# jerryli27/TwinGAN

Hardware: AMD Instinct MI355X
Metric: training images/sec (G+D step) at 256×256 final stage, 1/2/4/8 MI355X (higher is better)
Workload: dtype bf16; 1 GPU; TwinGAN 256x256 stage, batch 16 per GPU (configs[3]): E/G/2xD max_ch 256, UNet + per-domain instance norm + pixel norm, WGAN-GP, Adam; 1 step = G apply + D apply; global_batch=16, batch_per_gpu=16, parallelism=dp1, launch=hipGraph replay

## Files before the change

twingan_amd/csrc/norm.hip:

```cpp
#include "tg_common.h"
#include <stdlib.h>
#include <type_traits>

namespace {

#ifndef TG_NORM_BWD_U
#define TG_NORM_BWD_U 2
#endif
#define NF_LRELU 1
#define NF_PIXNORM 2
#define NF_ZEROSHIFT 8
#define NF_NOSTATS 4

template <typename T, int V>
struct VecIO {
  __device__ static __forceinline__ void load(const T* p, float* o) {
    if constexpr (V == 1) {
      o[0] = ld(p);
    } else {
      Vec16<T> v = ldv(p);
#pragma unroll
      for (int j = 0; j < V; ++j) o[j] = v.get(j);
    }
  }
// ... 447 lines not shown
        for (int q = 0; q < U; ++q) {
          const bool live = !TAIL || pb + q * lanes < p1;
          float yh[V];
          norm_act_gu<V>(gq[q], xq[q], sq[q], mu, rs, ga, be, flags, alpha, cv, inv_c, yh);
#pragma unroll
          for (int j = 0; j < V; ++j) {
            const float gr = live ? gq[q][j] : 0.f;
            a1[j] += gr;
            a2[j] = fmaf(gr, yh[j], a2[j]);
          }
        }
      }
    };
    if ((p1 - p0) % (lanes * U) == 0) sweep(std::false_type());
    else sweep(std::true_type());
  }
  wave_channel_accumulate<V>(a1, sh, 0, cv, v, pl < lanes);
  wave_channel_accumulate<V>(a2, sh, c, cv, v, pl < lanes);
  __syncthreads();
  float* out = sums + ((int64_t)n * gridDim.x + blockIdx.x) * 2 * c;
  for (int i = threadIdx.x; i < 2 * c; i += blockDim.x) out[i] = sh[i];
}

template <typename T, int V, int FL = -1>
__global__ void norm_act_bwd2_part_kernel(const T* __restrict__ gz, const T* __restrict__ gzp, int wdim,
                                          const T* __restrict__ y, const float* __restrict__ pn_scale,
                                          const float* __restrict__ mean, const float* __restrict__ rstd,
                                          const float* __restrict__ gamma, const float* __restrict__ beta,
                                          const float* __restrict__ gamma2, const float* __restrict__ beta2, int split,
                                          int pstride, T* __restrict__ gy, const float* __restrict__ part, int chunks,
                                          float* __restrict__ ggamma, float* __restrict__ gbeta,
                                          float* __restrict__ ggamma2, float* __restrict__ gbeta2, int sink, int hw, int c,
                                          int flags_rt, float alpha, int px_per_block) {
  extern __shared__ float sh[];
  const int flags = FL < 0 ? flags_rt : ((flags_rt & ~3) | FL);
  const int cv = c / V;
  const int lanes = blockDim.x / cv;
  const int v = threadIdx.x % cv, pl = threadIdx.x / cv;
  const int n = blockIdx.y;
  float mu[V], rs[V], ga[V], be[V];
#pragma unroll
  for (int j = 0; j < V; ++j) {
    const int ch = v * V + j;
    mu[j] = mean[n * c + ch];
    rs[j] = rstd[n * c + ch];
    ga[j] = pstride ? gamma[(int64_t)n * pstride + ch] : (n < split ? gamma : gamma2)[ch];
    be[j] = pstride ? beta[(int64_t)n * pstride + ch] : (n < split ? beta : beta2)[ch];
  }
  reduce_partials<exact_path<T>()>(part, n, chunks, c, sh);
  if (pstride && blockIdx.x == 0) {
    for (int i = threadIdx.x; i < c; i += blockDim.x) {
      if (gbeta) gbeta[(int64_t)n * pstride + i] = sh[i];
      if (ggamma) ggamma[(int64_t)n * pstride + i] = sh[c + i];
    }
  } else if (sink && blockIdx.x == 0) {
    float* gg = n < split ? ggamma : ggamma2;
    float* gb = n < split ? gbeta : gbeta2;
    if (sink == 2) {
      const int i0 = n < split ? 0 : split, i1 = n < split ? split : (int)gridDim.y;
      if (n == i0) {
        for (int i = threadIdx.x; i < 2 * c; i += blockDim.x) {
          float t = 0.f;
          const int64_t k1 = (int64_t)i1 * chunks;
          int64_t k = (int64_t)i0 * chunks;
          for (; k + 8 <= k1; k += 8) {
            float v[8];
#pragma unroll
            for (int u = 0; u < 8; ++u) v[u] = part[(k + u) * 2 * c + i];
#pragma unroll
            for (int u = 0; u < 8; ++u) t += v[u];
          }
          for (; k < k1; ++k) t += part[k * 2 * c + i];
          float* dst = i < c ? gb : gg;
          if (dst) atomicAdd(dst + (i < c ? i : i - c), t);
        }
      }
    } else {
      for (int i = threadIdx.x; i < c; i += blockDim.x) {
        if (gb) atomicAdd(gb + i, sh[i]);
        if (gg) atomicAdd(gg + i, sh[c + i]);
      }
    }
  }
  const float inv = 1.f / (float)hw;
  float s1[V], s2[V];
#pragma unroll
  for (int j = 0; j < V; ++j) {
    const int ch = v * V + j;
    s1[j] = (flags & NF_NOSTATS) ? 0.f : sh[ch] * inv;
    s2[j] = (flags & NF_NOSTATS) ? 0.f : sh[c + ch] * inv;
  }
  const int p0 = blockIdx.x * px_per_block;
  const int p1 = min(p0 + px_per_block, hw);
  if (pl >= lanes) return;
  const T* gz_n = gz ? gz + (int64_t)n * hw * c : nullptr;
  const T* gzp_n = gzp ? gzp + (int64_t)n * (hw >> 2) * c : nullptr;
  const T* y_n = y + (int64_t)n * hw * c;
  T* gy_n = gy + (int64_t)n * hw * c;
  const float* pn_n = pn_scale ? pn_scale + (int64_t)n * hw : nullptr;
  const int wshift = (wdim & (wdim - 1)) == 0 ? 31 - __builtin_clz(wdim) : -1;
  float gr[V];
#pragma unroll
  for (int j = 0; j < V; ++j) gr[j] = ga[j] * rs[j];
  const float inv_c = 1.f / (float)c;
  constexpr int U = TG_NORM_BWD_U;
  auto sweep = [&](auto tail) __attribute__((always_inline)) {
    constexpr bool TAIL = decltype(tail)::value;
    for (int pb = p0 + pl; pb < p1; pb += lanes * U) {
      float gq[U][V], xq[U][V], sq[U];
#pragma unroll
      for (int q = 0; q < U; ++q) {
        const unsigned p = TAIL ? min(pb + q * lanes, p1 - 1) : pb + q * lanes;
        load_grad_img<T, V>(gz_n, gzp_n, p, wshift, wdim, c, v, 0.25f, gq[q]);
        VecIO<T, V>::load(y_n + (p * c + v * V), xq[q]);
        sq[q] = (flags & NF_PIXNORM) ? pn_n[p] : 1.f;
      }
#pragma unroll
      for (int q = 0; q < U; ++q) {
        const unsigned p = pb + q * lanes;
        float yh[V];
        norm_act_gu<V>(gq[q], xq[q], sq[q], mu, rs, ga, be, flags, alpha, cv, inv_c, yh);
#pragma unroll
        for (int j = 0; j < V; ++j) gq[q][j] = gr[j] * (gq[q][j] - s1[j] - yh[j] * s2[j]);
        if (!TAIL || p < (unsigned)p1) VecIO<T, V>::store_stream(gy_n, p * c + v * V, gq[q]);
      }
    }
  };
  if ((p1 - p0) % (lanes * U) == 0) sweep(std::false_type());
  else sweep(std::true_type());
}

__global__ void norm_param_grads(const float* __restrict__ part, int chunks, float* __restrict__ ggamma,
                                 float* __restrict__ gbeta, float* __restrict__ ggamma2, float* __restrict__ gbeta2,
                                 int split, int n, int c, int accumulate) {
  const int ch = blockIdx.x * blockDim.x + threadIdx.x;
  if (ch >= c) return;
  const int i0 = blockIdx.y ? split : 0, i1 = blockIdx.y ? n : split;
  float* gg = blockIdx.y ? ggamma2 : ggamma;
  float* gb = blockIdx.y ? gbeta2 : gbeta;
  float sb = 0.f, sg = 0.f;
  for (int64_t k = (int64_t)i0 * chunks; k < (int64_t)i1 * chunks; ++k) {
    sb += part[k * 2 * c + ch];
    sg += part[k * 2 * c + c + ch];
  }
  if (gg) {
    if (accumulate) atomicAdd(gg + ch, sg);
    else gg[ch] = sg;
  }
  if (gb) {
    if (accumulate) atomicAdd(gb + ch, sb);
    else gb[ch] = sb;
  }
// ... 326 lines not shown
  norm_chunks(n, hw, &chunks, &ppb);
  int chunks2 = (2048 + n - 1) / n;
  int ppb2 = (hw + chunks2 - 1) / chunks2;
  if (ppb2 < min_ppb(hw)) ppb2 = min_ppb(hw);
  chunks2 = (hw + ppb2 - 1) / ppb2;
  const bool want_params = ggamma || gbeta || ggamma2 || gbeta2;
  TG_CHECK(!pstride || !accumulate, TG_EINVAL, "tg_norm_act_bwd: per-image parameter gradients are written, not added");
  int sink = (want_params && accumulate) ? 1 : 0;
  const size_t lds = 2 * (size_t)c * sizeof(float);
  TG_DISPATCH_DTYPE(dtype, "tg_norm_act_bwd", {
    if (sink && exact_grid<T>()) sink = 2;
    constexpr int VN = Vec16<T>::N;
    const bool vec = (c % VN == 0) && pow2(c / VN) && c / VN <= 64;
    if (flags & NF_PIXNORM) {
      TG_CHECK(vec && pn_scale, TG_ENOSUP, "tg_norm_act_bwd: pixel norm needs c (%d) = %d * 2^k and pn_scale", c, VN);
    }
    if (vec) {
      switch (flags & 3) {
        case 0: TG_NB_LAUNCH(0); break;
        case 1: TG_NB_LAUNCH(1); break;
        case 2: TG_NB_LAUNCH(2); break;
        default: TG_NB_LAUNCH(3); break;
      }
    } else {
      TG_CHECK(c <= 256, TG_ENOSUP, "tg_norm_act_bwd: scalar path needs c <= 256 (got %d)", c);
      hipLaunchKernelGGL((norm_act_bwd1_kernel<T, 1>), dim3(chunks, n), dim3(256), lds, s, (const T*)gz,
                         (const T*)gz_pooled, w, (const T*)y, pn_scale, mean, rstd, gamma, beta, gamma2, beta2, split, pstride, sums, hw, c, flags, alpha, ppb);
      hipLaunchKernelGGL((norm_act_bwd2_part_kernel<T, 1>), dim3(chunks2, n), dim3(256), lds, s, (const T*)gz,
                         (const T*)gz_pooled, w, (const T*)y, pn_scale, mean, rstd, gamma, beta, gamma2, beta2, split,
                         pstride, (T*)gy, sums, chunks, ggamma, gbeta, ggamma2, gbeta2, sink, hw, c, flags, alpha, ppb2);
    }
  });
  if (want_params && !sink && !pstride)
    hipLaunchKernelGGL(norm_param_grads, dim3((c + 255) / 256, split < n ? 2 : 1), dim3(256), 0, s, sums, chunks, ggamma,
                       gbeta, ggamma2, gbeta2, split, n, c, 0);
  TG_LAUNCH_CHECK("tg_norm_act_bwd");
  return TG_OK;
}

static int lrelu_bwd_launch(const char* who, const void* gz, const void* gzp, int hw, int wdim, const void* z, void* gy,
                            float* gbias, int64_t npix, int c, float alpha, int accumulate, int dtype, hipStream_t s,
                            bool z_is_sign_bits = false) {
  if (gbias && !accumulate) {
    int rc = tg_zero_async(gbias, (size_t)c * sizeof(float), nullptr, 0, s);
    if (rc) return rc;
  }
// ... 110 lines not shown
```

twingan_amd/csrc/pointwise.hip:

```cpp
#include "tg_common.h"

namespace {

template <typename T>
__global__ void axpby_kernel(const T* __restrict__ x, const T* __restrict__ y, T* __restrict__ out, int64_t numel, float a,
                             float b) {
  constexpr int V = Vec16<T>::N;
  const int64_t nvec = numel / V;
  const int64_t stride = (int64_t)gridDim.x * blockDim.x;
  for (int64_t i = (int64_t)blockIdx.x * blockDim.x + threadIdx.x; i < nvec; i += stride) {
    Vec16<T> vx = ldv(x + i * V), vo;
    if (y) {
      Vec16<T> vy = ldv(y + i * V);
#pragma unroll
      for (int j = 0; j < V; ++j) vo.set(j, a * vx.get(j) + b * vy.get(j));
    } else {
#pragma unroll
      for (int j = 0; j < V; ++j) vo.set(j, a * vx.get(j));
    }
    stv(out + i * V, vo);
  }
  for (int64_t i = nvec * V + (int64_t)blockIdx.x * blockDim.x + threadIdx.x; i < numel; i += stride)
    st(out + i, a * ld(x + i) + (y ? b * ld(y + i) : 0.f));
}
// ... 135 lines not shown
template <typename TS, typename TD>
__global__ void cast_kernel(const TS* __restrict__ s, TD* __restrict__ d, int64_t numel) {
  const int64_t stride = (int64_t)gridDim.x * blockDim.x;
  for (int64_t i = (int64_t)blockIdx.x * blockDim.x + threadIdx.x; i < numel; i += stride) st(d + i, ld(s + i));
}

template <typename T>
__global__ void sample_lerp_kernel(const T* __restrict__ x, const T* __restrict__ y, const float* __restrict__ alpha,
                                   T* __restrict__ out, int64_t per, int64_t numel) {
  const int64_t stride = (int64_t)gridDim.x * blockDim.x;
  for (int64_t i = (int64_t)blockIdx.x * blockDim.x + threadIdx.x; i < numel; i += stride) {
    const float a = alpha[i / per], vx = ld(x + i);
    st(out + i, vx + a * (ld(y + i) - vx));
  }
}

template <typename T>
__global__ void sample_scale_kernel(const T* __restrict__ x, const float* __restrict__ coef,
                                    const float* __restrict__ scalar, T* __restrict__ out, int64_t per, int64_t numel) {
  const int64_t stride = (int64_t)gridDim.x * blockDim.x;
  const float sc = scalar ? scalar[0] : 1.f;
  for (int64_t i = (int64_t)blockIdx.x * blockDim.x + threadIdx.x; i < numel; i += stride)
    st(out + i, ld(x + i) * coef[i / per] * sc);
}

template <typename T>
__global__ void gdrop_kernel(const T* __restrict__ x, const float* __restrict__ noise, const float* __restrict__ strength_dev,
                             float strength, float sqrt_c, T* __restrict__ out, int64_t per_image, int c, int64_t numel) {
  const int64_t stride = (int64_t)gridDim.x * blockDim.x;
  const float coef = (strength_dev ? strength_dev[0] : strength) * sqrt_c;
  for (int64_t i = (int64_t)blockIdx.x * blockDim.x + threadIdx.x; i < numel; i += stride) {
    const int64_t img = i / per_image;
    const int ch = (int)(i % c);
    st(out + i, ld(x + i) * fmaf(noise[img * c + ch], coef, 1.f));
  }
}

template <typename T, int V>
__global__ void upsample_concat_fwd_kernel(const T* __restrict__ x0, const T* __restrict__ x1, T* __restrict__ out, int n,
                                           int h, int w, int c0, int c1, int gsz, unsigned perm) {
  const int c = c0 + c1, cv = c / V, c0v = c0 / V;
  const int64_t total = (int64_t)n * (2 * h) * (2 * w) * cv;
  for (int64_t i = (int64_t)blockIdx.x * blockDim.x + threadIdx.x; i < total; i += (int64_t)gridDim.x * blockDim.x) {
    const int v = (int)(i % cv);
    int64_t p = i / cv;
    const int ox = (int)(p % (2 * w));
// ... 682 lines not shown
  else {
    tg_set_error("tg_cast: unsupported dtypes %d -> %d", sd, dd);
    return TG_EINVAL;
  }
  TG_LAUNCH_CHECK("tg_cast");
  return TG_OK;
}

int tg_sample_lerp(const void* x, const void* y, const float* alpha, void* out, int batch, int64_t per, int dtype,
                   void* stream) {
  TG_CHECK(x && y && alpha && out && batch > 0 && per > 0, TG_EINVAL, "tg_sample_lerp: bad arguments");
  TG_DISPATCH_DTYPE(dtype, "tg_sample_lerp", {
    hipLaunchKernelGGL(sample_lerp_kernel<T>, dim3(tg_grid_for(batch * per, 256)), dim3(256), 0, (hipStream_t)stream,
                       (const T*)x, (const T*)y, alpha, (T*)out, per, batch * per);
  });
  TG_LAUNCH_CHECK("tg_sample_lerp");
  return TG_OK;
}

int tg_sample_scale(const void* x, const float* coef, const float* scalar, void* out, int batch, int64_t per, int dtype,
                    void* stream) {
  TG_CHECK(x && coef && out && batch > 0 && per > 0, TG_EINVAL, "tg_sample_scale: bad arguments");
  TG_DISPATCH_DTYPE(dtype, "tg_sample_scale", {
    hipLaunchKernelGGL(sample_scale_kernel<T>, dim3(tg_grid_for(batch * per, 256)), dim3(256), 0, (hipStream_t)stream,
                       (const T*)x, coef, scalar, (T*)out, per, batch * per);
  });
  TG_LAUNCH_CHECK("tg_sample_scale");
  return TG_OK;
}

int tg_gdrop(const void* x, const float* noise, const float* strength_dev, float strength, int c_logical, void* out, int n,
             int64_t hw, int c, int dtype, void* stream) {
  TG_CHECK(x && noise && out && n > 0 && hw > 0 && c > 0 && c_logical > 0 && c_logical <= c, TG_EINVAL, "tg_gdrop: bad arguments");
  const int64_t per = hw * c;
  TG_DISPATCH_DTYPE(dtype, "tg_gdrop", {
    hipLaunchKernelGGL(gdrop_kernel<T>, dim3(tg_grid_for(n * per, 256)), dim3(256), 0, (hipStream_t)stream, (const T*)x, noise,
                       strength_dev, strength, sqrtf((float)c_logical), (T*)out, per, c, n * per);
  });
  TG_LAUNCH_CHECK("tg_gdrop");
  return TG_OK;
}

#define TG_SPATIAL_LAUNCH(KERNEL, VECOK, TOTAL_VEC, TOTAL_SCALAR, ...)                                                 \
  TG_DISPATCH_DTYPE(dtype, #KERNEL, {                                                                                  \
    constexpr int V = Vec16<T>::N;                                                                                     \
    if (VECOK(V))                                                                                                      \
      hipLaunchKernelGGL((KERNEL<T, V>), dim3(tg_grid_for(TOTAL_VEC(V), 256)), dim3(256), 0, (hipStream_t)stream,      \
                         __VA_ARGS__);                                                                                 \
// ... 149 lines not shown
```

twingan_amd/csrc/reduce.hip:

```cpp
#include "tg_common.h"

namespace {

constexpr int MB_NMAX = 16;
template <typename T, int V>
struct alignas(sizeof(T) * V) MbVec {
  T e[V];
  __device__ __forceinline__ float get(int i) const { return (float)e[i]; }
  __device__ __forceinline__ void set(int i, float x) { e[i] = (T)x; }
};
template <typename T> constexpr int mb_v() { return 8 / (int)sizeof(T); }
template <typename T, int V> __device__ __forceinline__ MbVec<T, V> mb_ld(const T* p) {
  return *reinterpret_cast<const MbVec<T, V>*>(p);
}
template <typename T, int V> __device__ __forceinline__ void mb_st(T* p, const MbVec<T, V>& v) {
  *reinterpret_cast<MbVec<T, V>*>(p) = v;
}
template <typename T, int V>
__device__ __forceinline__ void mb_load_samples(const T* __restrict__ x, int n, int P, int p, MbVec<T, V> (&xv)[MB_NMAX]) {
#pragma unroll
  for (int i = 0; i < MB_NMAX; ++i) xv[i] = mb_ld<T, V>(x + (int64_t)(i < n ? i : n - 1) * P + p);
}


// ... 348 lines not shown
      mb_copy_with_stat<T, 9>(v, ggout, total / V16, c, cpad, Tt);
    } else {
      for (int64_t i = threadIdx.x; i < total; i += blockDim.x) {
        const int ch = (int)(i % cpad);
        const int64_t px = i / cpad;
        float o = 0.f;
        if (ch < c)
          o = ld(v + px * c + ch);
        else if (ch == c)
          o = Tt;
        st(ggout + i, o);
      }
    }
  }
}

template <typename T, int MODE, bool PART = false>
__global__ void sum_kernel(const T* __restrict__ x, const T* __restrict__ y, float* __restrict__ out, int64_t numel,
                           float scale, int direct = 0, int vec = 1) {
  __shared__ float red[8];
  constexpr int V = Vec16<T>::N;
  const int64_t nvec = vec ? numel / V : 0, stride = (int64_t)gridDim.x * blockDim.x;
  float acc = 0.f;
  for (int64_t i = (int64_t)blockIdx.x * blockDim.x + threadIdx.x; i < nvec; i += stride) {
    Vec16<T> a = ldv(x + i * V);
    if (MODE == 0) {
#pragma unroll
      for (int j = 0; j < V; ++j) acc += a.get(j);
    } else {
      Vec16<T> b = ldv(y + i * V);
#pragma unroll
      for (int j = 0; j < V; ++j) acc += fabsf(a.get(j) - b.get(j));
    }
  }
  for (int64_t i = nvec * V + (int64_t)blockIdx.x * blockDim.x + threadIdx.x; i < numel; i += stride)
    acc += MODE == 0 ? ld(x + i) : fabsf(ld(x + i) - ld(y + i));
  const float tot = block_sum(acc, red);
  if (threadIdx.x == 0) {
    if constexpr (PART) out[blockIdx.x] = tot;
    else if (direct) out[0] = tot * scale;
    else atomicAdd(out, tot * scale);
  }
}

__global__ void ordered_scalar_sum_kernel(const float* __restrict__ part, int n, float* __restrict__ out, float scale,
                                          int accumulate) {
  if (blockIdx.x || threadIdx.x) return;
  float t = 0.f;
  for (int i = 0; i < n; ++i) t += part[i];
  out[0] = accumulate ? out[0] + t * scale : t * scale;
}

template <typename T>
__global__ void abs_diff_bwd_kernel(const T* __restrict__ a, const T* __restrict__ b, const float* __restrict__ gscale,
                                    T* __restrict__ ga, T* __restrict__ gb, int64_t numel, float scale) {
  const float g = (gscale ? gscale[0] : 1.f) * scale;
  for (int64_t i = (int64_t)blockIdx.x * blockDim.x + threadIdx.x; i < numel; i += (int64_t)gridDim.x * blockDim.x) {
    const float d = ld(a + i) - ld(b + i);
    const float s = d > 0.f ? g : (d < 0.f ? -g : 0.f);
    if (ga) st(ga + i, s);
    if (gb) st(gb + i, -s);
  }
}

template <typename T>
__global__ void sample_sumsq_kernel(const T* __restrict__ x, float* __restrict__ out, int64_t per, int vec) {
  __shared__ float red[8];
  constexpr int V = Vec16<T>::N;
  const T* base = x + (int64_t)blockIdx.y * per;
  const int64_t nvec = vec ? per / V : 0, stride = (int64_t)gridDim.x * blockDim.x;
  float acc = 0.f;
  for (int64_t i = (int64_t)blockIdx.x * blockDim.x + threadIdx.x; i < nvec; i += stride) {
    Vec16<T> a = ldv(base + i * V);
#pragma unroll
    for (int j = 0; j < V; ++j) acc = fmaf(a.get(j), a.get(j), acc);
  }
  for (int64_t i = nvec * V + (int64_t)blockIdx.x * blockDim.x + threadIdx.x; i < per; i += stride) {
    const float a = ld(base + i);
    acc = fmaf(a, a, acc);
  }
  const float tot = block_sum(acc, red);
  if (threadIdx.x == 0) atomicAdd(out + blockIdx.y, tot);
}

__global__ void gp_penalty_kernel(const float* __restrict__ ss, float* __restrict__ loss, float* __restrict__ coef,
                                  int batch, float lambda) {
  __shared__ float red[8];
  float acc = 0.f;
  for (int b = threadIdx.x; b < batch; b += blockDim.x) {
    const float slope = sqrtf(ss[b]);
    const float d = slope - 1.f;
    acc += d * d;
    if (coef) coef[b] = slope > 0.f ? lambda * 2.f * d / (slope * (float)batch) : 0.f;
  }
  const float tot = block_sum(acc, red);
  if (threadIdx.x == 0 && loss) loss[0] = lambda * tot / (float)batch;
}

// ... 147 lines not shown
template <typename T>
__global__ void fc_bwd_kernel(const T* __restrict__ x, const float* __restrict__ w, const float* __restrict__ g,
                              T* __restrict__ gx, float* __restrict__ gw, float* __restrict__ gb, int m, int n, int k,
                              int acc_w, int acc_b) {
  const int kk = blockIdx.x * blockDim.x + threadIdx.x;
  if (kk < k) {
    for (int row = 0; gx && row < m; ++row) {
      float a = 0.f;
      for (int col = 0; col < n; ++col) a = fmaf(g[(int64_t)row * n + col], w[(int64_t)kk * n + col], a);
      st(gx + (int64_t)row * k + kk, a);
    }
    for (int col = 0; gw && col < n; ++col) {
      float a = 0.f;
      for (int row = 0; row < m; ++row) a = fmaf(ld(x + (int64_t)row * k + kk), g[(int64_t)row * n + col], a);
      gw[(int64_t)kk * n + col] = (acc_w ? gw[(int64_t)kk * n + col] : 0.f) + a;
    }
  }
  if (gb && kk < n) {
    float a = 0.f;
    for (int row = 0; row < m; ++row) a += g[(int64_t)row * n + kk];
    gb[kk] = (acc_b ? gb[kk] : 0.f) + a;
  }
}

__global__ void small_gemm_kernel(const float* __restrict__ a, const float* __restrict__ b, const float* __restrict__ bias,
                                  float* __restrict__ c, int m, int n, int k, int ta, int tb, int accumulate) {
  const int64_t total = (int64_t)m * n;
  for (int64_t i = (int64_t)blockIdx.x * blockDim.x + threadIdx.x; i < total; i += (int64_t)gridDim.x * blockDim.x) {
    const int col = (int)(i % n), row = (int)(i / n);
    float acc = 0.f;
    for (int kk = 0; kk < k; ++kk) {
      const float av = ta ? a[(int64_t)kk * m + row] : a[(int64_t)row * k + kk];
      const float bv = tb ? b[(int64_t)col * k + kk] : b[(int64_t)kk * n + col];
      acc = fmaf(av, bv, acc);
    }
    if (bias) acc += bias[col];
    c[i] = (accumulate ? c[i] : 0.f) + acc;
  }
}

__global__ void small_gemm_wave_kernel(const float* __restrict__ a, const float* __restrict__ b,
                                       const float* __restrict__ bias, float* __restrict__ c, int m, int n, int k, int ta,
                                       int tb, int accumulate) {
  const int64_t total = (int64_t)m * n;
  const int lane = threadIdx.x & 63;
  const int64_t w0 = ((int64_t)blockIdx.x * blockDim.x + threadIdx.x) >> 6, nw = ((int64_t)gridDim.x * blockDim.x) >> 6;
// ... 61 lines not shown
    int nsplit = (hw * c / mb_v<T>() + 255) / 256;
    if (nsplit < 1) nsplit = 1;
    if (nsplit > 8) nsplit = 8;
    hipLaunchKernelGGL(mbstd_bwd_kernel<T>, dim3(groups, nsplit), dim3(256), 0, (hipStream_t)stream, (const T*)gout, (const T*)x,
                       (T*)gx, n / groups, hw, c, cpad, eps);
  });
  TG_LAUNCH_CHECK("tg_mbstd_bwd");
  return TG_OK;
}

int tg_mbstd_bwd_bwd(const void* v, const void* gout, const void* x, void* ggout, void* gx2, int n, int groups, int hw, int c,
                     int cpad, float eps, int dtype, void* stream) {
  TG_CHECK(v && gout && x && n > 0 && hw > 0 && c > 0 && cpad > c, TG_EINVAL, "tg_mbstd_bwd_bwd: bad arguments");
  TG_CHECK(groups > 0 && n % groups == 0, TG_EINVAL, "tg_mbstd_bwd_bwd: n (%d) not divisible by groups (%d)", n, groups);
  TG_DISPATCH_DTYPE(dtype, "tg_mbstd_bwd_bwd", {
    constexpr int NTHR = sizeof(T) == 4 ? 512 : 1024;
    hipLaunchKernelGGL((mbstd_bwd_bwd_kernel<T, NTHR>), dim3(groups), dim3(NTHR), 0, (hipStream_t)stream, (const T*)v,
                       (const T*)gout, (const T*)x, (T*)ggout, (T*)gx2, n / groups, hw, c, cpad, eps);
  });
  TG_LAUNCH_CHECK("tg_mbstd_bwd_bwd");
  return TG_OK;
}

static int zero_unless(float* p, size_t bytes, int accumulate, hipStream_t s, const char* who) {
  if (!accumulate) return tg_zero_async(p, bytes, nullptr, 0, s);
  return TG_OK;
}

int tg_sum(const void* x, float* out, int64_t numel, float scale, int accumulate, int dtype, void* stream) {
  TG_CHECK(x && out && numel > 0, TG_EINVAL, "tg_sum: bad arguments");
  hipStream_t s = (hipStream_t)stream;
  TG_DISPATCH_DTYPE(dtype, "tg_sum", {
    const int blocks = exact_grid<T>() ? 1 : tg_grid_for(numel / Vec16<T>::N + 1, 256, 1024);
    const int direct = (blocks == 1 && !accumulate) ? 1 : 0;
    if (!direct) {
      int rc = zero_unless(out, sizeof(float), accumulate, s, "tg_sum");
      if (rc) return rc;
    }
    hipLaunchKernelGGL((sum_kernel<T, 0>), dim3(blocks), dim3(256), 0, s, (const T*)x, (const T*)nullptr, out, numel, scale, direct,
                       tg_aligned16(x));
  });
  TG_LAUNCH_CHECK("tg_sum");
  return TG_OK;
}

int tg_abs_diff_sum(const void* a, const void* b, float* out, int64_t numel, float scale, int accumulate, int dtype,
                    void* stream) {
  TG_CHECK(a && b && out && numel > 0, TG_EINVAL, "tg_abs_diff_sum: bad arguments");
  hipStream_t s = (hipStream_t)stream;
  TG_DISPATCH_DTYPE(dtype, "tg_abs_diff_sum", {
    const int blocks = exact_grid<T>() ? 1 : tg_grid_for(numel / Vec16<T>::N + 1, 256, 1024);
    const int direct = (blocks == 1 && !accumulate) ? 1 : 0;
    if (!direct) {
      int rc = zero_unless(out, sizeof(float), accumulate, s, "tg_abs_diff_sum");
      if (rc) return rc;
    }
    hipLaunchKernelGGL((sum_kernel<T, 1>), dim3(blocks), dim3(256), 0, s, (const T*)a, (const T*)b, out, numel, scale, direct,
                       tg_aligned16(a) && tg_aligned16(b));
  });
  TG_LAUNCH_CHECK("tg_abs_diff_sum");
  return TG_OK;
}

int tg_sum_ordered(const void* x, const void* y_or_null, float* out, int64_t numel, float scale, int accumulate, float* ws,
                   size_t ws_floats, int dtype, void* stream) {
  TG_CHECK(x && out && ws && ws_floats >= 1 && numel > 0, TG_EINVAL, "tg_sum_ordered: bad arguments");
  hipStream_t s = (hipStream_t)stream;
  int blocks = 0;
  TG_DISPATCH_DTYPE(dtype, "tg_sum_ordered", {
    blocks = tg_grid_for(numel / Vec16<T>::N + 1, 256, 512);
    if ((size_t)blocks > ws_floats) blocks = (int)ws_floats;
    if (y_or_null)
      hipLaunchKernelGGL((sum_kernel<T, 1, true>), dim3(blocks), dim3(256), 0, s, (const T*)x, (const T*)y_or_null, ws, numel, 1.f, 0,
                         tg_aligned16(x) && tg_aligned16(y_or_null));
// ... 3 lines not shown
  });
  hipLaunchKernelGGL(ordered_scalar_sum_kernel, dim3(1), dim3(64), 0, s, ws, blocks, out, scale, accumulate);
  TG_LAUNCH_CHECK("tg_sum_ordered");
  return TG_OK;
}

int tg_abs_diff_bwd(const void* a, const void* b, const float* gscale, void* ga, void* gb, int64_t numel, float scale,
                    int dtype, void* stream) {
  TG_CHECK(a && b && numel > 0 && (ga || gb), TG_EINVAL, "tg_abs_diff_bwd: bad arguments");
  TG_DISPATCH_DTYPE(dtype, "tg_abs_diff_bwd", {
    hipLaunchKernelGGL(abs_diff_bwd_kernel<T>, dim3(tg_grid_for(numel, 256)), dim3(256), 0, (hipStream_t)stream,
                       (const T*)a, (const T*)b, gscale, (T*)ga, (T*)gb, numel, scale);
  });
  TG_LAUNCH_CHECK("tg_abs_diff_bwd");
  return TG_OK;
}

int tg_sample_sumsq(const void* x, float* out, int batch, int64_t per, int dtype, void* stream) {
  TG_CHECK(x && out && batch > 0 && per > 0, TG_EINVAL, "tg_sample_sumsq: bad arguments");
  hipStream_t s = (hipStream_t)stream;
  int rc = zero_unless(out, (size_t)batch * sizeof(float), 0, s, "tg_sample_sumsq");
  if (rc) return rc;
  TG_DISPATCH_DTYPE(dtype, "tg_sample_sumsq", {
    const int chunks = exact_grid<T>() ? 1 : tg_grid_for(per / Vec16<T>::N + 1, 256, 64);
    const int vec = tg_aligned16(x) && (batch == 1 || per % Vec16<T>::N == 0);
    hipLaunchKernelGGL(sample_sumsq_kernel<T>, dim3(chunks, batch), dim3(256), 0, s, (const T*)x, out, per, vec);
  });
  TG_LAUNCH_CHECK("tg_sample_sumsq");
  return TG_OK;
}

int tg_gp_penalty(const float* sumsq, float* loss, float* coef, int batch, float lambda, void* stream) {
  TG_CHECK(sumsq && batch > 0, TG_EINVAL, "tg_gp_penalty: bad arguments");
  hipLaunchKernelGGL(gp_penalty_kernel, dim3(1), dim3(256), 0, (hipStream_t)stream, sumsq, loss, coef, batch, lambda);
  TG_LAUNCH_CHECK("tg_gp_penalty");
  return TG_OK;
}

int tg_pred_loss_fwd(const float* x, float* out, int n, int mode, float a, float b, float scale, int accumulate,
                     void* stream) {
  TG_CHECK(x && out && n > 0 && mode >= 0 && mode <= 3, TG_EINVAL, "tg_pred_loss_fwd: bad arguments");
  hipLaunchKernelGGL(pred_loss_fwd_kernel, dim3(1), dim3(256), 0, (hipStream_t)stream, x, out, n, mode, a, b, scale,
                     accumulate);
  TG_LAUNCH_CHECK("tg_pred_loss_fwd");
  return TG_OK;
}

// ... 89 lines not shown
    hipLaunchKernelGGL(small_gemm_wave_kernel, dim3(tg_grid_for((int64_t)m * n * 64, 256)), dim3(256), 0,
                       (hipStream_t)stream, a, b, bias, c, m, n, k, ta, tb, accumulate);
  else
    hipLaunchKernelGGL(small_gemm_kernel, dim3(tg_grid_for((int64_t)m * n, 256)), dim3(256), 0, (hipStream_t)stream, a, b,
                       bias, c, m, n, k, ta, tb, accumulate);
  TG_LAUNCH_CHECK("tg_small_gemm");
  return TG_OK;
}

int tg_fc_fwd(const void* x, const float* w, const float* bias, float* y, int m, int n, int k, int dtype, void* stream) {
  TG_CHECK(x && w && y && m > 0 && n > 0 && k > 0, TG_EINVAL, "tg_fc_fwd: bad arguments");
  TG_DISPATCH_DTYPE(dtype, "tg_fc_fwd", {
    hipLaunchKernelGGL(fc_fwd_kernel<T>, dim3(tg_grid_for((int64_t)m * n * 64, 256)), dim3(256), 0, (hipStream_t)stream,
                       (const T*)x, w, bias, y, m, n, k);
  });
  TG_LAUNCH_CHECK("tg_fc_fwd");
  return TG_OK;
}

int tg_fc_bwd(const void* x, const float* w, const float* g, void* gx, float* gw, float* gb, int m, int n, int k, int acc_w,
              int acc_b, int dtype, void* stream) {
  TG_CHECK(x && w && g && (gx || gw || gb) && m > 0 && n > 0 && k > 0 && n <= k, TG_EINVAL, "tg_fc_bwd: bad arguments");
  TG_DISPATCH_DTYPE(dtype, "tg_fc_bwd", {
    hipLaunchKernelGGL(fc_bwd_kernel<T>, dim3(tg_grid_for(k, 64)), dim3(64), 0, (hipStream_t)stream, (const T*)x, w, g, (T*)gx,
                       gw, gb, m, n, k, acc_w, acc_b);
  });
  TG_LAUNCH_CHECK("tg_fc_bwd");
  return TG_OK;
}

int tg_adam_step(float* theta, const float* grad, float* m, float* v, void* theta_bf16, int64_t numel, float lr_t,
                 const float* lr_t_dev, float beta1, float beta2, float eps, float grad_scale, void* stream) {
  TG_CHECK(theta && grad && m && v && numel > 0, TG_EINVAL, "tg_adam_step: bad arguments");
  hipLaunchKernelGGL(adam_kernel, dim3(tg_grid_for(numel, 256)), dim3(256), 0, (hipStream_t)stream, theta, grad, m, v,
                     (bf16*)theta_bf16, numel, lr_t, lr_t_dev, beta1, beta2, eps, grad_scale);
  TG_LAUNCH_CHECK("tg_adam_step");
  return TG_OK;
}

int tg_adam_tick(int64_t* step_dev, float* lr_t_dev, float lr, float beta1, float beta2, void* stream) {
  TG_CHECK(step_dev && lr_t_dev, TG_EINVAL, "tg_adam_tick: null pointer");
  hipLaunchKernelGGL(adam_tick_kernel, dim3(1), dim3(64), 0, (hipStream_t)stream, step_dev, lr_t_dev, lr, beta1, beta2);
  TG_LAUNCH_CHECK("tg_adam_tick");
  return TG_OK;
}

}
```

Baseline: 1090 images/sec.

## Add specialized RGB norm backward, vectorized sample scale, unrolled reductions, wave fc_bwd

Adds dedicated kernels for the 3-channel (RGB) instance-norm backward that process four pixels per thread with 8-byte vector loads, replacing the scalar c<=256 fallback. It also vectorizes the per-sample scale kernel, unrolls the sum, abs-diff and sumsq reductions by four with a wider-grid heuristic, and replaces the bf16 fc backward with a multi-wave kernel that splits the weight, input and bias gradients across blocks. These target memory-bound small kernels and poorly occupied launches. They add code paths gated on alignment and dtype, and they change the reduction order.

Result: no change. 1097 images/sec, median of 5 (+0.6%).

```diff
diff --git a/twingan_amd/csrc/norm.hip b/twingan_amd/csrc/norm.hip
--- a/twingan_amd/csrc/norm.hip
+++ b/twingan_amd/csrc/norm.hip
@@ -493,6 +493,46 @@
   for (int i = threadIdx.x; i < 2 * c; i += blockDim.x) out[i] = sh[i];
 }
 
+__device__ __forceinline__ void norm_bwd2_param_grads(const float* __restrict__ part, int chunks, const float* sh, int n, int c,
+                                                      int pstride, int sink, int split, float* __restrict__ ggamma,
+                                                      float* __restrict__ gbeta, float* __restrict__ ggamma2,
+                                                      float* __restrict__ gbeta2) {
+  if (pstride && blockIdx.x == 0) {
+    for (int i = threadIdx.x; i < c; i += blockDim.x) {
+      if (gbeta) gbeta[(int64_t)n * pstride + i] = sh[i];
+      if (ggamma) ggamma[(int64_t)n * pstride + i] = sh[c + i];
+    }
+  } else if (sink && blockIdx.x == 0) {
+    float* gg = n < split ? ggamma : ggamma2;
+    float* gb = n < split ? gbeta : gbeta2;
+    if (sink == 2) {
+      const int i0 = n < split ? 0 : split, i1 = n < split ? split : (int)gridDim.y;
+      if (n == i0) {
+        for (int i = threadIdx.x; i < 2 * c; i += blockDim.x) {
+          float t = 0.f;
+          const int64_t k1 = (int64_t)i1 * chunks;
+          int64_t k = (int64_t)i0 * chunks;
+          for (; k + 8 <= k1; k += 8) {
+            float v[8];
+#pragma unroll
+            for (int u = 0; u < 8; ++u) v[u] = part[(k + u) * 2 * c + i];
+#pragma unroll
+            for (int u = 0; u < 8; ++u) t += v[u];
+          }
+          for (; k < k1; ++k) t += part[k * 2 * c + i];
+          float* dst = i < c ? gb : gg;
+          if (dst) atomicAdd(dst + (i < c ? i : i - c), t);
+        }
+      }
+    } else {
+      for (int i = threadIdx.x; i < c; i += blockDim.x) {
+        if (gb) atomicAdd(gb + i, sh[i]);
+        if (gg) atomicAdd(gg + i, sh[c + i]);
+      }
+    }
+  }
+}
+
 template <typename T, int V, int FL = -1>
 __global__ void norm_act_bwd2_part_kernel(const T* __restrict__ gz, const T* __restrict__ gzp, int wdim,
                                           const T* __restrict__ y, const float* __restrict__ pn_scale,
@@ -519,40 +559,7 @@
     be[j] = pstride ? beta[(int64_t)n * pstride + ch] : (n < split ? beta : beta2)[ch];
   }
   reduce_partials<exact_path<T>()>(part, n, chunks, c, sh);
-  if (pstride && blockIdx.x == 0) {
-    for (int i = threadIdx.x; i < c; i += blockDim.x) {
-      if (gbeta) gbeta[(int64_t)n * pstride + i] = sh[i];
-      if (ggamma) ggamma[(int64_t)n * pstride + i] = sh[c + i];
-    }
-  } else if (sink && blockIdx.x == 0) {
-    float* gg = n < split ? ggamma : ggamma2;
-    float* gb = n < split ? gbeta : gbeta2;
-    if (sink == 2) {
-      const int i0 = n < split ? 0 : split, i1 = n < split ? split : (int)gridDim.y;
-      if (n == i0) {
-        for (int i = threadIdx.x; i < 2 * c; i += blockDim.x) {
-          float t = 0.f;
-          const int64_t k1 = (int64_t)i1 * chunks;
-          int64_t k = (int64_t)i0 * chunks;
-          for (; k + 8 <= k1; k += 8) {
-            float v[8];
-#pragma unroll
-            for (int u = 0; u < 8; ++u) v[u] = part[(k + u) * 2 * c + i];
-#pragma unroll
-            for (int u = 0; u < 8; ++u) t += v[u];
-          }
-          for (; k < k1; ++k) t += part[k * 2 * c + i];
-          float* dst = i < c ? gb : gg;
-          if (dst) atomicAdd(dst + (i < c ? i : i - c), t);
-        }
-      }
-    } else {
-      for (int i = threadIdx.x; i < c; i += blockDim.x) {
-        if (gb) atomicAdd(gb + i, sh[i]);
-        if (gg) atomicAdd(gg + i, sh[c + i]);
-      }
-    }
-  }
+  norm_bwd2_param_grads(part, chunks, sh, n, c, pstride, sink, split, ggamma, gbeta, ggamma2, gbeta2);
   const float inv = 1.f / (float)hw;
   float s1[V], s2[V];
 #pragma unroll
@@ -599,6 +606,161 @@
   };
   if ((p1 - p0) % (lanes * U) == 0) sweep(std::false_type());
   else sweep(std::true_type());
+}
+
+template <typename T> struct Quad16;
+template <> struct Quad16<bf16> { typedef bf16x4 type; };
+template <> struct Quad16<f16> { typedef __attribute__((ext_vector_type(4))) _Float16 type; };
+template <> struct Quad16<float> { typedef f32x4 type; };
+
+struct Rgb3Consts {
+  float mu[3], rs[3], ga[3], be[3];
+};
+__device__ __forceinline__ Rgb3Consts rgb3_consts(const float* __restrict__ mean, const float* __restrict__ rstd,
+                                                  const float* __restrict__ gamma, const float* __restrict__ beta,
+                                                  const float* __restrict__ gamma2, const float* __restrict__ beta2, int split,
+                                                  int pstride, int n) {
+  Rgb3Consts k;
+#pragma unroll
+  for (int ch = 0; ch < 3; ++ch) {
+    k.mu[ch] = mean[n * 3 + ch];
+    k.rs[ch] = rstd[n * 3 + ch];
+    k.ga[ch] = pstride ? gamma[(int64_t)n * pstride + ch] : (n < split ? gamma : gamma2)[ch];
+    k.be[ch] = pstride ? beta[(int64_t)n * pstride + ch] : (n < split ? beta : beta2)[ch];
+  }
+  return k;
+}
+template <typename T>
+__device__ __forceinline__ void rgb3_load_quad(const T* img, unsigned q, typename Quad16<T>::type (&o)[3]) {
+  const typename Quad16<T>::type* sp = reinterpret_cast<const typename Quad16<T>::type*>(img + q * 12u);
+#pragma unroll
+  for (int w = 0; w < 3; ++w) o[w] = sp[w];
+}
+template <typename T>
+__device__ __forceinline__ void rgb3_gu(const typename Quad16<T>::type (&gq)[3], const typename Quad16<T>::type (&yq)[3],
+                                        bool have_gz, const T* gzp_n, unsigned q, unsigned wdim, const Rgb3Consts& k,
+                                        int flags, float alpha, float (&g)[12], float (&yh)[12]) {
+#pragma unroll
+  for (int e = 0; e < 12; ++e) g[e] = have_gz ? (float)gq[e >> 2][e & 3] : 0.f;
+  if (gzp_n) {
+#pragma unroll
+    for (int px = 0; px < 4; ++px) {
+      const unsigned p = 4 * q + px, yy = p / wdim, xx = p - yy * wdim;
+      const T* cell = gzp_n + ((yy >> 1) * (wdim >> 1) + (xx >> 1)) * 3u;
+#pragma unroll
+      for (int ch = 0; ch < 3; ++ch) g[px * 3 + ch] = fmaf(0.25f, ld(cell + ch), g[px * 3 + ch]);
+    }
+  }
+#pragma unroll
+  for (int e = 0; e < 12; ++e) {
+    const int ch = e % 3;
+    yh[e] = ((float)yq[e >> 2][e & 3] - k.mu[ch]) * k.rs[ch];
+    const float u = yh[e] * k.ga[ch] + k.be[ch];
+    if ((flags & NF_LRELU) && !(u > 0.f)) g[e] *= alpha;
+  }
+}
+
+template <typename T>
+__global__ __launch_bounds__(256) void norm_act_bwd1_rgb4_kernel(
+    const T* __restrict__ gz, const T* __restrict__ gzp, int wdim, const T* __restrict__ y, const float* __restrict__ mean,
+    const float* __restrict__ rstd, const float* __restrict__ gamma, const float* __restrict__ beta,
+    const float* __restrict__ gamma2, const float* __restrict__ beta2, int split, int pstride, float* __restrict__ sums, int hw,
+    int flags, float alpha, int q_per_block) {
+  typedef typename Quad16<T>::type q16;
+  constexpr int U = 2;
+  __shared__ float red[4][6];
+  const int n = blockIdx.y;
+  const Rgb3Consts k = rgb3_consts(mean, rstd, gamma, beta, gamma2, beta2, split, pstride, n);
+  const T* gz_n = gz ? gz + (int64_t)n * hw * 3 : nullptr;
+  const T* gzp_n = gzp ? gzp + (int64_t)n * (hw >> 2) * 3 : nullptr;
+  const T* y_n = y + (int64_t)n * hw * 3;
+  const int q0 = blockIdx.x * q_per_block, q1 = min(q0 + q_per_block, hw >> 2);
+  float a[6];
+#pragma unroll
+  for (int i = 0; i < 6; ++i) a[i] = 0.f;
+  for (int qb = q0 + (int)threadIdx.x; qb < q1; qb += 256 * U) {
+    q16 gq[U][3], yq[U][3];
+#pragma unroll
+    for (int u = 0; u < U; ++u) {
+      const unsigned q = min(qb + u * 256, q1 - 1);
+      if (gz_n) rgb3_load_quad<T>(gz_n, q, gq[u]);
+      rgb3_load_quad<T>(y_n, q, yq[u]);
+    }
+#pragma unroll
+    for (int u = 0; u < U; ++u) {
+      const bool live = qb + u * 256 < q1;
+      float g[12], yh[12];
+      rgb3_gu<T>(gq[u], yq[u], gz_n != nullptr, gzp_n, min(qb + u * 256, q1 - 1), wdim, k, flags, alpha, g, yh);
+#pragma unroll
+      for (int e = 0; e < 12; ++e) {
+        const float gr = live ? g[e] : 0.f;
+        a[e % 3] += gr;
+        a[3 + e % 3] = fmaf(gr, yh[e], a[3 + e % 3]);
+      }
+    }
+  }
+  const int lane = threadIdx.x & 63, wave = threadIdx.x >> 6;
+#pragma unroll
+  for (int i = 0; i < 6; ++i) {
+    a[i] = wave_sum(a[i]);
+    if (lane == 0) red[wave][i] = a[i];
+  }
+  __syncthreads();
+  if (threadIdx.x < 6)
+    sums[((int64_t)n * gridDim.x + blockIdx.x) * 6 + threadIdx.x] =
+        ((red[0][threadIdx.x] + red[1][threadIdx.x]) + red[2][threadIdx.x]) + red[3][threadIdx.x];
+}
+
+template <typename T>
+__global__ __launch_bounds__(256) void norm_act_bwd2_rgb4_kernel(
+    const T* __restrict__ gz, const T* __restrict__ gzp, int wdim, const T* __restrict__ y, const float* __restrict__ mean,
+    const float* __restrict__ rstd, const float* __restrict__ gamma, const float* __restrict__ beta,
+    const float* __restrict__ gamma2, const float* __restrict__ beta2, int split, int pstride, T* __restrict__ gy,
+    const float* __restrict__ part, int chunks, float* __restrict__ ggamma, float* __restrict__ gbeta,
+    float* __restrict__ ggamma2, float* __restrict__ gbeta2, int sink, int hw, int flags, float alpha, int q_per_block) {
+  typedef typename Quad16<T>::type q16;
+  constexpr int U = 2;
+  __shared__ float sh[6];
+  const int n = blockIdx.y;
+  const Rgb3Consts k = rgb3_consts(mean, rstd, gamma, beta, gamma2, beta2, split, pstride, n);
+  reduce_partials<false>(part, n, chunks, 3, sh);
+  norm_bwd2_param_grads(part, chunks, sh, n, 3, pstride, sink, split, ggamma, gbeta, ggamma2, gbeta2);
+  const float inv = 1.f / (float)hw;
+  float s1[3], s2[3], gr[3];
+#pragma unroll
+  for (int ch = 0; ch < 3; ++ch) {
+    s1[ch] = (flags & NF_NOSTATS) ? 0.f : sh[ch] * inv;
+    s2[ch] = (flags & NF_NOSTATS) ? 0.f : sh[3 + ch] * inv;
+    gr[ch] = k.ga[ch] * k.rs[ch];
+  }
+  const T* gz_n = gz ? gz + (int64_t)n * hw * 3 : nullptr;
+  const T* gzp_n = gzp ? gzp + (int64_t)n * (hw >> 2) * 3 : nullptr;
+  const T* y_n = y + (int64_t)n * hw * 3;
+  T* gy_n = gy + (int64_t)n * hw * 3;
+  const int q0 = blockIdx.x * q_per_block, q1 = min(q0 + q_per_block, hw >> 2);
+  for (int qb = q0 + (int)threadIdx.x; qb < q1; qb += 256 * U) {
+    q16 gq[U][3], yq[U][3];
+#pragma unroll
+    for (int u = 0; u < U; ++u) {
+      const unsigned q = min(qb + u * 256, q1 - 1);
+      if (gz_n) rgb3_load_quad<T>(gz_n, q, gq[u]);
+      rgb3_load_quad<T>(y_n, q, yq[u]);
+    }
+#pragma unroll
+    for (int u = 0; u < U; ++u) {
+      const unsigned q = min(qb + u * 256, q1 - 1);
+      float g[12], yh[12];
+      rgb3_gu<T>(gq[u], yq[u], gz_n != nullptr, gzp_n, q, wdim, k, flags, alpha, g, yh);
+      q16 o[3];
+#pragma unroll
+      for (int e = 0; e < 12; ++e) o[e >> 2][e & 3] = (T)(gr[e % 3] * (g[e] - s1[e % 3] - yh[e] * s2[e % 3]));
+      if (qb + u * 256 < q1) {
+        q16* dp = reinterpret_cast<q16*>(gy_n + q * 12u);
+#pragma unroll
+        for (int w = 0; w < 3; ++w) dp[w] = o[w];
+      }
+    }
+  }
 }
 
 __global__ void norm_param_grads(const float* __restrict__ part, int chunks, float* __restrict__ ggamma,
@@ -971,6 +1133,14 @@
         case 2: TG_NB_LAUNCH(2); break;
         default: TG_NB_LAUNCH(3); break;
       }
+    } else if (sizeof(T) == 2 && c == 3 && hw % 4 == 0 && !(flags & NF_PIXNORM) &&
+               ((reinterpret_cast<uintptr_t>(gz) | reinterpret_cast<uintptr_t>(y) | reinterpret_cast<uintptr_t>(gy)) & 7u) == 0) {
+      const int nq = hw / 4, qpb = (nq + chunks - 1) / chunks, qpb2 = (nq + chunks2 - 1) / chunks2;
+      hipLaunchKernelGGL(norm_act_bwd1_rgb4_kernel<T>, dim3(chunks, n), dim3(256), 0, s, (const T*)gz, (const T*)gz_pooled, w,
+                         (const T*)y, mean, rstd, gamma, beta, gamma2, beta2, split, pstride, sums, hw, flags, alpha, qpb);
+      hipLaunchKernelGGL(norm_act_bwd2_rgb4_kernel<T>, dim3(chunks2, n), dim3(256), 0, s, (const T*)gz, (const T*)gz_pooled, w,
+                         (const T*)y, mean, rstd, gamma, beta, gamma2, beta2, split, pstride, (T*)gy, sums, chunks, ggamma, gbeta,
+                         ggamma2, gbeta2, sink, hw, flags, alpha, qpb2);
     } else {
       TG_CHECK(c <= 256, TG_ENOSUP, "tg_norm_act_bwd: scalar path needs c <= 256 (got %d)", c);
       hipLaunchKernelGGL((norm_act_bwd1_kernel<T, 1>), dim3(chunks, n), dim3(256), lds, s, (const T*)gz,
diff --git a/twingan_amd/csrc/pointwise.hip b/twingan_amd/csrc/pointwise.hip
--- a/twingan_amd/csrc/pointwise.hip
+++ b/twingan_amd/csrc/pointwise.hip
@@ -181,6 +181,32 @@
   const float sc = scalar ? scalar[0] : 1.f;
   for (int64_t i = (int64_t)blockIdx.x * blockDim.x + threadIdx.x; i < numel; i += stride)
     st(out + i, ld(x + i) * coef[i / per] * sc);
+}
+template <typename T>
+__global__ void sample_scale_vec_kernel(const T* __restrict__ x, const float* __restrict__ coef,
+                                        const float* __restrict__ scalar, T* __restrict__ out, int64_t pervec, int64_t nvec) {
+  constexpr int V = Vec16<T>::N, U = 4;
+  const int64_t stride = (int64_t)gridDim.x * blockDim.x;
+  const float sc = scalar ? scalar[0] : 1.f;
+  for (int64_t i = (int64_t)blockIdx.x * blockDim.x + threadIdx.x; i < nvec; i += stride * U) {
+    Vec16<T> a[U];
+    float cf[U];
+#pragma unroll
+    for (int u = 0; u < U; ++u) {
+      const int64_t iu = i + u * stride < nvec ? i + u * stride : nvec - 1;
+      a[u] = ldv(x + iu * V);
+      cf[u] = coef[iu / pervec];
+    }
+#pragma unroll
+    for (int u = 0; u < U; ++u) {
+      if (i + u * stride < nvec) {
+        Vec16<T> o;
+#pragma unroll
+        for (int j = 0; j < V; ++j) o.set(j, a[u].get(j) * cf[u] * sc);
+        stv(out + (i + u * stride) * V, o);
+      }
+    }
+  }
 }
 
 template <typename T>
@@ -909,8 +935,15 @@
                     void* stream) {
   TG_CHECK(x && coef && out && batch > 0 && per > 0, TG_EINVAL, "tg_sample_scale: bad arguments");
   TG_DISPATCH_DTYPE(dtype, "tg_sample_scale", {
-    hipLaunchKernelGGL(sample_scale_kernel<T>, dim3(tg_grid_for(batch * per, 256)), dim3(256), 0, (hipStream_t)stream,
-                       (const T*)x, coef, scalar, (T*)out, per, batch * per);
+    constexpr int V = Vec16<T>::N;
+    if (per % V == 0 && tg_aligned16(x) && tg_aligned16(out)) {
+      const int64_t nvec = batch * per / V;
+      hipLaunchKernelGGL(sample_scale_vec_kernel<T>, dim3(tg_grid_for(nvec, 256 * 4)), dim3(256), 0, (hipStream_t)stream,
+                         (const T*)x, coef, scalar, (T*)out, per / V, nvec);
+    } else {
+      hipLaunchKernelGGL(sample_scale_kernel<T>, dim3(tg_grid_for(batch * per, 256)), dim3(256), 0, (hipStream_t)stream,
+                         (const T*)x, coef, scalar, (T*)out, per, batch * per);
+    }
   });
   TG_LAUNCH_CHECK("tg_sample_scale");
   return TG_OK;
diff --git a/twingan_amd/csrc/reduce.hip b/twingan_amd/csrc/reduce.hip
--- a/twingan_amd/csrc/reduce.hip
+++ b/twingan_amd/csrc/reduce.hip
@@ -394,15 +394,26 @@
   constexpr int V = Vec16<T>::N;
   const int64_t nvec = vec ? numel / V : 0, stride = (int64_t)gridDim.x * blockDim.x;
   float acc = 0.f;
-  for (int64_t i = (int64_t)blockIdx.x * blockDim.x + threadIdx.x; i < nvec; i += stride) {
-    Vec16<T> a = ldv(x + i * V);
-    if (MODE == 0) {
-#pragma unroll
-      for (int j = 0; j < V; ++j) acc += a.get(j);
-    } else {
-      Vec16<T> b = ldv(y + i * V);
-#pragma unroll
-      for (int j = 0; j < V; ++j) acc += fabsf(a.get(j) - b.get(j));
+  constexpr int U = 4;
+  for (int64_t i = (int64_t)blockIdx.x * blockDim.x + threadIdx.x; i < nvec; i += stride * U) {
+    Vec16<T> a[U], b[U];
+#pragma unroll
+    for (int u = 0; u < U; ++u) {
+      const int64_t iu = i + u * stride < nvec ? i + u * stride : nvec - 1;
+      a[u] = ldv(x + iu * V);
+      if constexpr (MODE != 0) b[u] = ldv(y + iu * V);
+    }
+#pragma unroll
+    for (int u = 0; u < U; ++u) {
+      if (i + u * stride < nvec) {
+        if (MODE == 0) {
+#pragma unroll
+          for (int j = 0; j < V; ++j) acc += a[u].get(j);
+        } else {
+#pragma unroll
+          for (int j = 0; j < V; ++j) acc += fabsf(a[u].get(j) - b[u].get(j));
+        }
+      }
     }
   }
   for (int64_t i = nvec * V + (int64_t)blockIdx.x * blockDim.x + threadIdx.x; i < numel; i += stride)
@@ -442,10 +453,18 @@
   const T* base = x + (int64_t)blockIdx.y * per;
   const int64_t nvec = vec ? per / V : 0, stride = (int64_t)gridDim.x * blockDim.x;
   float acc = 0.f;
-  for (int64_t i = (int64_t)blockIdx.x * blockDim.x + threadIdx.x; i < nvec; i += stride) {
-    Vec16<T> a = ldv(base + i * V);
-#pragma unroll
-    for (int j = 0; j < V; ++j) acc = fmaf(a.get(j), a.get(j), acc);
+  constexpr int U = 4;
+  for (int64_t i = (int64_t)blockIdx.x * blockDim.x + threadIdx.x; i < nvec; i += stride * U) {
+    Vec16<T> a[U];
+#pragma unroll
+    for (int u = 0; u < U; ++u) a[u] = ldv(base + (i + u * stride < nvec ? i + u * stride : nvec - 1) * V);
+#pragma unroll
+    for (int u = 0; u < U; ++u) {
+      if (i + u * stride < nvec) {
+#pragma unroll
+        for (int j = 0; j < V; ++j) acc = fmaf(a[u].get(j), a[u].get(j), acc);
+      }
+    }
   }
   for (int64_t i = nvec * V + (int64_t)blockIdx.x * blockDim.x + threadIdx.x; i < per; i += stride) {
     const float a = ld(base + i);
@@ -639,6 +658,47 @@
     gb[kk] = (acc_b ? gb[kk] : 0.f) + a;
   }
 }
+template <typename T>
+__global__ __launch_bounds__(256) void fc_bwd_wave_kernel(const T* __restrict__ x, const float* __restrict__ w,
+                                                          const float* __restrict__ g, T* __restrict__ gx,
+                                                          float* __restrict__ gw, float* __restrict__ gb, int m, int n, int k,
+                                                          int acc_w, int acc_b, int nbw, int nbx) {
+  const int lane = threadIdx.x & 63, wave = threadIdx.x >> 6;
+  int blk = blockIdx.x;
+  if (blk < nbw) {
+    const int kk = (blk * 4 + wave) * 8 + (lane & 7), rl = lane >> 3;
+    const bool live = kk < k;
+    const int kc = live ? kk : k - 1;
+    for (int col = 0; col < n; ++col) {
+      float a = 0.f;
+#pragma unroll 8
+      for (int row = rl; row < m; row += 8) a = fmaf(ld(x + (int64_t)row * k + kc), g[(int64_t)row * n + col], a);
+#pragma unroll
+      for (int o = 8; o < 64; o <<= 1) a += __shfl_xor(a, o, 64);
+      if (live && rl == 0) gw[(int64_t)kk * n + col] = (acc_w ? gw[(int64_t)kk * n + col] : 0.f) + a;
+    }
+    return;
+  }
+  blk -= nbw;
+  if (blk < nbx) {
+    const int64_t total = (int64_t)m * k;
+    for (int64_t i = (int64_t)blk * blockDim.x + threadIdx.x; i < total; i += (int64_t)nbx * blockDim.x) {
+      const int row = (int)(i / k), kk = (int)(i - (int64_t)row * k);
+      float a = 0.f;
+      for (int col = 0; col < n; ++col) a = fmaf(g[(int64_t)row * n + col], w[(int64_t)kk * n + col], a);
+      st(gx + i, a);
+    }
+    return;
+  }
+  if (gb && wave == 0) {
+    for (int col = 0; col < n; ++col) {
+      float a = 0.f;
+      for (int row = lane; row < m; row += 64) a += g[(int64_t)row * n + col];
+      a = wave_sum(a);
+      if (lane == 0) gb[col] = (acc_b ? gb[col] : 0.f) + a;
+    }
+  }
+}
 
 __global__ void small_gemm_kernel(const float* __restrict__ a, const float* __restrict__ b, const float* __restrict__ bias,
                                   float* __restrict__ c, int m, int n, int k, int ta, int tb, int accumulate) {
@@ -746,6 +806,13 @@
   return TG_OK;
 }
 
+static inline int sum_grid(int64_t nvec, int cap, int slices) {
+  const int narrow = tg_grid_for(nvec, 256, cap);
+  if (narrow < cap) return narrow;
+  const int wide = tg_grid_for(nvec, 256 * 4, cap);
+  return (int64_t)wide * slices >= 256 ? wide : narrow;
+}
+
 static int zero_unless(float* p, size_t bytes, int accumulate, hipStream_t s, const char* who) {
   if (!accumulate) return tg_zero_async(p, bytes, nullptr, 0, s);
   return TG_OK;
@@ -755,7 +822,7 @@
   TG_CHECK(x && out && numel > 0, TG_EINVAL, "tg_sum: bad arguments");
   hipStream_t s = (hipStream_t)stream;
   TG_DISPATCH_DTYPE(dtype, "tg_sum", {
-    const int blocks = exact_grid<T>() ? 1 : tg_grid_for(numel / Vec16<T>::N + 1, 256, 1024);
+    const int blocks = exact_grid<T>() ? 1 : sum_grid(numel / Vec16<T>::N + 1, 1024, 1);
     const int direct = (blocks == 1 && !accumulate) ? 1 : 0;
     if (!direct) {
       int rc = zero_unless(out, sizeof(float), accumulate, s, "tg_sum");
@@ -773,7 +840,7 @@
   TG_CHECK(a && b && out && numel > 0, TG_EINVAL, "tg_abs_diff_sum: bad arguments");
   hipStream_t s = (hipStream_t)stream;
   TG_DISPATCH_DTYPE(dtype, "tg_abs_diff_sum", {
-    const int blocks = exact_grid<T>() ? 1 : tg_grid_for(numel / Vec16<T>::N + 1, 256, 1024);
+    const int blocks = exact_grid<T>() ? 1 : sum_grid(numel / Vec16<T>::N + 1, 1024, 1);
     const int direct = (blocks == 1 && !accumulate) ? 1 : 0;
     if (!direct) {
       int rc = zero_unless(out, sizeof(float), accumulate, s, "tg_abs_diff_sum");
@@ -823,7 +890,7 @@
   int rc = zero_unless(out, (size_t)batch * sizeof(float), 0, s, "tg_sample_sumsq");
   if (rc) return rc;
   TG_DISPATCH_DTYPE(dtype, "tg_sample_sumsq", {
-    const int chunks = exact_grid<T>() ? 1 : tg_grid_for(per / Vec16<T>::N + 1, 256, 64);
+    const int chunks = exact_grid<T>() ? 1 : sum_grid(per / Vec16<T>::N + 1, 64, batch);
     const int vec = tg_aligned16(x) && (batch == 1 || per % Vec16<T>::N == 0);
     hipLaunchKernelGGL(sample_sumsq_kernel<T>, dim3(chunks, batch), dim3(256), 0, s, (const T*)x, out, per, vec);
   });
@@ -959,8 +1026,14 @@
               int acc_b, int dtype, void* stream) {
   TG_CHECK(x && w && g && (gx || gw || gb) && m > 0 && n > 0 && k > 0 && n <= k, TG_EINVAL, "tg_fc_bwd: bad arguments");
   TG_DISPATCH_DTYPE(dtype, "tg_fc_bwd", {
-    hipLaunchKernelGGL(fc_bwd_kernel<T>, dim3(tg_grid_for(k, 64)), dim3(64), 0, (hipStream_t)stream, (const T*)x, w, g, (T*)gx,
-                       gw, gb, m, n, k, acc_w, acc_b);
+    if constexpr (exact_path<T>()) {
+      hipLaunchKernelGGL(fc_bwd_kernel<T>, dim3(tg_grid_for(k, 64)), dim3(64), 0, (hipStream_t)stream, (const T*)x, w, g, (T*)gx,
+                         gw, gb, m, n, k, acc_w, acc_b);
+    } else {
+      const int nbw = gw ? tg_grid_for(k, 32) : 0, nbx = gx ? tg_grid_for((int64_t)m * k, 256, 256) : 0, nbb = gb ? 1 : 0;
+      hipLaunchKernelGGL(fc_bwd_wave_kernel<T>, dim3(nbw + nbx + nbb), dim3(256), 0, (hipStream_t)stream, (const T*)x, w, g,
+                         (T*)gx, gw, gb, m, n, k, acc_w, acc_b, nbw, nbx);
+    }
   });
   TG_LAUNCH_CHECK("tg_fc_bwd");
   return TG_OK;
```
